# kekoveca/MPI-and-Open-MP

Measured on AMD Instinct MI355X. Metric: Gcell-updates/sec at 1/2/4/8 MI355X + % of HBM roofline, bit-exact, higher is better.
Workload: dtype u32 (1 bit/cell)

## Files before the change

include/life_mi355x.h:

```cpp
#ifndef LIFE_MI355X_H
#define LIFE_MI355X_H

#include <stdint.h>

#ifdef __cplusplus
extern "C" {
#endif

#define LIFE_OK 0
#define LIFE_EINVAL (-1)
#define LIFE_EHIP (-2)
#define LIFE_ERCCL (-3)
#define LIFE_ENOMEM (-4)
#define LIFE_ESTATE (-5)
#define LIFE_EIO (-6)

#define LIFE_KERNEL_BYTE 0
#define LIFE_KERNEL_BIT 1

#define LIFE_XPORT_AUTO 0
#define LIFE_XPORT_RCCL 1
#define LIFE_XPORT_LOCAL 2

typedef struct life_dev life_dev;
// ... 76 lines not shown

int life_dev_gather_bits(life_dev *d, uint8_t *packed);

int64_t life_dev_live_count(life_dev *d);

int life_dev_checksum(life_dev *d, uint64_t *sum);


int life_dev_clear(life_dev *d);

int life_dev_set_cells(life_dev *d, const int64_t *xy, int64_t n, int alive);

int life_dev_gather_rect(life_dev *d, int64_t x0, int64_t y0, int64_t w, int64_t h, uint8_t *cells);

int life_dev_gather_density(life_dev *d, int64_t fx, int64_t fy, uint32_t *counts);

int life_dev_sync(life_dev *d);
int life_dev_barrier(life_dev *d);
int life_device_count(void);
int life_dev_layout(life_dev *d, int local_shard, life_layout *out);
int life_dev_world(life_dev *d, int *world, int *dims0, int *dims1, int *nlocal, int *transport);
int life_dev_shard_info(life_dev *d, int local_shard, int *device, char pci_bus_id[64], int *rccl_nranks);

int life_dev_set_timing(life_dev *d, int on);

#define LIFE_OPT_SMALL_GRID 1
#define LIFE_OPT_OVERLAP 2
#define LIFE_OPT_BLOCK_GENS 5
#define LIFE_OPT_SMALL_WINDOW 4
#define LIFE_OPT_LOOPBACK 6
#define LIFE_OPT_FLOW 7
#define LIFE_OPT_FLOW_CHUNK 8
#define LIFE_OPT_DEEP_HALO 9
int life_dev_configure(life_dev *d, int option, int value);
#define LIFE_PATH_NONE 0
#define LIFE_PATH_ONEGEN 1
#define LIFE_PATH_TILES 2
#define LIFE_PATH_FLOW 3
#define LIFE_PATH_SMALL 5
int life_dev_last_path(life_dev *d);
int life_dev_kernel_stats(life_dev *d, double *avg_ms, int64_t *launches, double *bytes_per_launch);
int life_dev_kernel_work(life_dev *d, double *cell_updates_per_launch, double *valu_ops_per_launch);
int life_dev_phase_stats(life_dev *d, double *ring_ms, double *interior_ms, double *halo_ms, double *block_ms,
                         int64_t *blocks);
int life_dev_call_stats(life_dev *d, double *host_enqueue_ms, double *pass_enqueue_max_ms, int64_t *passes,
                        double *device_span_ms);

int life_tune(int kernel, int rows, int depth);

int life_tune_temporal(int kernel, int rows);

int life_measure_copy(int device, int64_t bytes, int reps, double *gbps);

void life_dev_destroy(life_dev *d);

#ifdef __cplusplus
}
#endif
#endif
```

mpi-and-open-mp_amd/csrc/life_dev.hip:

```cpp
#include <stdarg.h>

#include <chrono>
#include <thread>

#include "life_dev_internal.h"
#include "life_env.h"

using namespace life::rt;

thread_local std::string life::rt::g_err;

void life::rt::set_err(const char *fmt, ...) {
    char buf[512];
    va_list ap;
    va_start(ap, fmt);
    vsnprintf(buf, sizeof buf, fmt, ap);
    va_end(ap);
    g_err = buf;
}

static const int kEnvBlockGens = life::env::read(life::env::kBlockGens);
static const int kEnvFlow = life::env::read(life::env::kFlow);
static const bool kEnvDeepHalo = life::env::read(life::env::kDeepHalo) != 0;
static int default_block_gens(int kernel) {
    return kEnvBlockGens ? kEnvBlockGens : (kernel == LIFE_KERNEL_BIT ? 12 : 32);
}

namespace {

int alloc_fill_byte() { return life::env::read(life::env::kPoison) ? 0xA5 : 0; }

int shard_alloc(Shard &s) {
    HIPCHK(hipSetDevice(s.device));
    HIPCHK(hipStreamCreateWithPriority(&s.stream, hipStreamNonBlocking, 0));
    HIPCHK(hipStreamCreateWithPriority(&s.stream2, hipStreamNonBlocking, 0));
    HIPCHK(hipStreamCreateWithPriority(&s.comm_stream, hipStreamNonBlocking, 0));
    const int fill = alloc_fill_byte();
    const int64_t slack = s.lay.generations_per_exchange > 1 ? life::kTemporalSlackRows : 0;
    const size_t bytes = (size_t)(s.lay.pitch * (s.lay.rows + slack));
    for (int i = 0; i < 2; i++) {
        HIPCHK(hipMalloc(&s.buf[i], bytes));
        HIPCHK(hipMemsetAsync(s.buf[i], fill, bytes, s.stream));
    }
    HIPCHK(hipEventCreateWithFlags(&s.ev_int, hipEventDisableTiming));
    HIPCHK(hipEventCreateWithFlags(&s.ev_halo, hipEventDisableTiming));
    HIPCHK(hipEventCreateWithFlags(&s.ev_sync, hipEventDisableTiming));
    HIPCHK(hipEventCreateWithFlags(&s.ev_entry, hipEventDisableTiming));
    const size_t col_bytes = (size_t)life::column_stage_bytes(s.lay);
    HIPCHK(hipMalloc(&s.col_send, col_bytes));
    HIPCHK(hipMalloc(&s.col_recv, col_bytes));
    HIPCHK(hipMalloc(&s.d_count, 2 * sizeof(unsigned long long)));
    HIPCHK(hipMalloc(&s.sink, 1024));
    HIPCHK(hipMemsetAsync(s.col_send, fill, col_bytes, s.stream));
    HIPCHK(hipMemsetAsync(s.col_recv, fill, col_bytes, s.stream));
    HIPCHK(hipMemsetAsync(s.d_count, 0, 2 * sizeof(unsigned long long), s.stream));
    HIPCHK(hipMemsetAsync(s.sink, fill, 1024, s.stream));
    HIPCHK(hipStreamSynchronize(s.stream));
    HIPCHK(hipHostMalloc(&s.h_count, 2 * sizeof *s.h_count, hipHostMallocDefault));
    return LIFE_OK;
}

void shard_free(Shard &s) {
    (void)hipSetDevice(s.device);
    if (s.comm) (void)ncclCommDestroy(s.comm);
    for (auto &t : s.timers) {
        if (t.a) (void)hipEventDestroy(t.a);
        if (t.b) (void)hipEventDestroy(t.b);
    }
    for (auto &p : s.phases)
        for (hipEvent_t e : {p.ring0, p.ring1, p.int0, p.int1, p.halo0, p.halo1, p.end})
            if (e) (void)hipEventDestroy(e);
    for (uint8_t *p : {s.buf[0], s.buf[1], s.col_send, s.col_recv, s.sink, s.stage})
        if (p) (void)hipFree(p);
    if (s.flow) (void)hipFree(s.flow);
    if (s.d_count) (void)hipFree(s.d_count);
    if (s.h_count) (void)hipHostFree(s.h_count);
    for (hipEvent_t e : {s.ev_halo, s.ev_sync, s.ev_int, s.ev_entry, s.own_a, s.own_b})
        if (e) (void)hipEventDestroy(e);
    if (s.stream) (void)hipStreamDestroy(s.stream);
    if (s.stream2) (void)hipStreamDestroy(s.stream2);
    if (s.comm_stream) (void)hipStreamDestroy(s.comm_stream);
}

double comm_timeout_s() {
    static const double t = life::env::read(life::env::kCommTimeoutS);
    return t;
}

int agree_all_ranks(life_dev *d, int value, const char *what) {
    for (Shard &s : d->shards) {
        if (!s.comm) continue;
        HIPCHK(hipSetDevice(s.device));
        int64_t *h = reinterpret_cast<int64_t *>(s.h_count);
        h[0] = value;
        h[1] = -(int64_t)value;
        HIPCHK(hipMemcpyAsync(s.d_count, h, 2 * sizeof(int64_t), hipMemcpyHostToDevice, s.stream));
        NCCLCHK(ncclAllReduce(s.d_count, s.d_count, 2, ncclInt64, ncclMax, s.comm, s.stream));
        HIPCHK(hipMemcpyAsync(h, s.d_count, 2 * sizeof(int64_t), hipMemcpyDeviceToHost, s.stream));
        CHK(bounded_sync(s, what, -1));
        const int64_t hi = h[0], lo = -h[1];
        if (hi != lo) {
            set_err("%s is collective in rank mode: ranks passed %lld .. %lld", what, (long long)lo, (long long)hi);
            return LIFE_EINVAL;
        }
    }
    return LIFE_OK;
}

life_dev *new_dev(int64_t nx, int64_t ny, int dims0, int dims1, int world, int kernel) {
    int dims[2] = {dims0, dims1};
    if (dims0 <= 0 || dims1 <= 0) life_dims_create(world, dims);
    if (dims[0] * dims[1] != world) return nullptr;
    life_dev *d = new life_dev;
    d->nx = nx;
    d->ny = ny;
    d->dims[0] = dims[0];
    d->dims[1] = dims[1];
    d->world = world;
    d->kernel = kernel;
    d->block_gens = default_block_gens(kernel);
    d->deep = kEnvDeepHalo;
    d->flow = kEnvFlow;
    return d;
}

int create_shards(life_dev *d, const std::vector<int> &ranks, const std::vector<int> &devices) {
    for (size_t i = 0; i < ranks.size(); i++) {
        d->shards.emplace_back();
        Shard &s = d->shards.back();
        s.rank = ranks[i];
        s.device = devices[i];
        const int rc = life_layout_query(d->nx, d->ny, d->dims[0], d->dims[1], s.rank, d->kernel, &s.lay);
        if (rc != LIFE_OK) {
            set_err("layout: nx=%lld ny=%lld dims=%dx%d rank %d kernel %d", (long long)d->nx,
                    (long long)d->ny, d->dims[0], d->dims[1], s.rank, d->kernel);
            return rc;
        }
    }
    for (Shard &s : d->shards) CHK(shard_alloc(s));
    return plan_halos(d);
}

void tail_prewarm(const life_dev *d) {
    for (size_t i = 0; i < d->shards.size(); ++i) {
        bool seen = false;
        for (size_t j = 0; j < i; ++j)
            seen |= d->shards[j].lay.w == d->shards[i].lay.w && d->shards[j].lay.h == d->shards[i].lay.h;
        if (!seen) life::prewarm_tail_plans(d->shards[i].lay, max_pass_gens(d), part(d, 1));
    }
}

int finish_create(life_dev *d, int rc, life_dev **out) {
    if (rc != LIFE_OK) {
        life_dev_destroy(d);
        return rc;
// ... 232 lines not shown
    if (!d) return LIFE_EINVAL;
    CHK(life_dev_sync(d));
    switch (option) {
    case LIFE_OPT_SMALL_GRID:
        if (value < 0 || value > 4) return LIFE_EINVAL;
        d->small_mode = value;
        return LIFE_OK;
    case LIFE_OPT_SMALL_WINDOW: {
        const int R = value >> 8, K = value & 255;
        if (value != 0 && (K < 1 || R < 1 || R > 8 || R == 7)) return LIFE_EINVAL;
        if (value != 0 && life::reg_win_plan(d->shards[0].lay, R, K).blocks == 0) {
            set_err("small-grid window R=%d K=%d does not fit this grid", R, K);
            return LIFE_EINVAL;
        }
        d->win_rows = R;
        d->win_halo = K;
        return LIFE_OK;
    }
    case LIFE_OPT_OVERLAP: d->overlap = value != 0; return LIFE_OK;
    case LIFE_OPT_BLOCK_GENS:
        if (value < 0 || value > 32) return LIFE_EINVAL;
        d->block_gens = value > 0 ? value : default_block_gens(d->kernel);
        tail_prewarm(d);
        return LIFE_OK;
    case LIFE_OPT_FLOW:
        if (value < 0 || value > 3) return LIFE_EINVAL;
        d->flow = value;
        return LIFE_OK;
    case LIFE_OPT_DEEP_HALO:
        if (value < 0 || value > 1) return LIFE_EINVAL;
        if (d->rank_mode && d->world > 1) CHK(agree_all_ranks(d, value, "LIFE_OPT_DEEP_HALO"));
        d->deep = value != 0;
        return LIFE_OK;
    case LIFE_OPT_FLOW_CHUNK:
        if (value < 0) return LIFE_EINVAL;
        d->flow_chunk = value;
        return LIFE_OK;
    case LIFE_OPT_LOOPBACK: {
        if (value < 0 || value > 3) return LIFE_EINVAL;
        if (d->world != 1 || d->shards.size() != 1) {
            set_err("loopback needs a single-shard world (world %d, %zu local shards)", d->world, d->shards.size());
            return LIFE_EINVAL;
        }
        Shard &s = d->shards[0];
        if (value && (s.lay.h < s.lay.yapron || s.lay.w < s.lay.xapron)) {
            set_err("loopback: %lld x %lld cells < the %lld-column / %lld-row halo", (long long)s.lay.w,
                    (long long)s.lay.h, (long long)s.lay.xapron, (long long)s.lay.yapron);
            return LIFE_EINVAL;
        }
        if (value && d->transport == LIFE_XPORT_RCCL && !s.comm) {
            set_err("loopback over RCCL needs a communicator (life_dev_create_rank with a unique id, or "
                    "life_dev_create_ex with LIFE_XPORT_RCCL)");
            return LIFE_EINVAL;
        }
        d->loop = value == 0 ? 0 : value == 1 ? 3 : value == 2 ? 1 : 2;
        CHK(plan_halos(d));
        CHK(exchange(d, 0, false));
        tail_prewarm(d);
        return life_dev_sync(d);
    }
    default: return LIFE_EINVAL;
    }
}

int life_tune(int kernel, int rows, int depth) {
    if ((rows && rows != 16 && rows != 32 && rows != 64) ||
// ... 20 lines not shown
```

mpi-and-open-mp_amd/csrc/life_dev_internal.h:

```cpp
#pragma once
#include <rccl/rccl.h>
#include <stdio.h>
#include <string.h>

#include <algorithm>
#include <string>
#include <vector>

#include "life_host.h"
#include "life_io.h"
#include "life_kernels.h"
#include "life_mi355x.h"

#pragma GCC visibility push(hidden)

namespace life {
namespace rt {

extern thread_local std::string g_err;
void set_err(const char *fmt, ...);

#define HIPCHK(expr)                                                                          \
    do {                                                                                      \
        hipError_t e_ = (expr);                                                               \
        if (e_ != hipSuccess) {                                                               \
            life::rt::set_err("%s:%d %s: %s", __FILE__, __LINE__, #expr, hipGetErrorString(e_)); \
            return e_ == hipErrorOutOfMemory ? LIFE_ENOMEM : LIFE_EHIP;                       \
        }                                                                                     \
    } while (0)

#define NCCLCHK(expr)                                                                         \
    do {                                                                                      \
        ncclResult_t r_ = (expr);                                                             \
        if (r_ != ncclSuccess) {                                                              \
            life::rt::set_err("%s:%d %s: %s", __FILE__, __LINE__, #expr, ncclGetErrorString(r_)); \
            return LIFE_ERCCL;                                                                \
        }                                                                                     \
    } while (0)

#define CHK(expr)                     \
    do {                              \
        int rc_ = (expr);             \
        if (rc_ != LIFE_OK) return rc_; \
    } while (0)

struct TimedLaunch {
    hipEvent_t a = nullptr, b = nullptr;
    int launches = 1;
};

struct PhaseEvents {
    hipEvent_t ring0 = nullptr, ring1 = nullptr, int0 = nullptr, int1 = nullptr, halo0 = nullptr,
               halo1 = nullptr, end = nullptr;
};

struct LocalCopy {
    int phase, src, sop, sslot, dop, dslot;
    size_t bytes;
};

struct Shard {
    int rank = 0;
    int device = 0;
    life_layout lay{};
    uint8_t *buf[2] = {nullptr, nullptr};
    int cur = 0;
    hipStream_t stream = nullptr;
    hipStream_t stream2 = nullptr;
    hipStream_t comm_stream = nullptr;
    hipEvent_t ev_halo = nullptr, ev_sync = nullptr, ev_int = nullptr;
    hipEvent_t ev_entry = nullptr;
    hipEvent_t own_a = nullptr, own_b = nullptr, span_a = nullptr, span_b = nullptr;
    ncclComm_t comm = nullptr;
    uint8_t *col_send = nullptr, *col_recv = nullptr;
    unsigned long long *d_count = nullptr;
    unsigned long long *h_count = nullptr;
    uint8_t *sink = nullptr;
    uint8_t *stage = nullptr;
    size_t stage_bytes = 0;
    unsigned int *flow = nullptr;
    size_t flow_words = 0;
    bool flow_used = false;
    std::vector<life_halo_op> plan;
    bool corners = false;
    std::vector<int> slot;
    std::vector<LocalCopy> copies;
    std::vector<int> waits[2][2];
    std::vector<TimedLaunch> timers;
    size_t timers_used = 0;
    std::vector<PhaseEvents> phases;
    size_t phases_used = 0;
};

}
}

struct life_dev {
    int64_t nx = 0, ny = 0;
    int dims[2] = {1, 1};
    int world = 1;
    int kernel = LIFE_KERNEL_BYTE;
    int transport = LIFE_XPORT_LOCAL;
    bool rank_mode = false;
    bool timing = false;
    bool phase_events = true;
    bool launch_events = true;
    bool overlap = true;
    int block_gens = 0;
    int small_mode = 1;
    int win_rows = 0, win_halo = 0;
    int loop = 0;
    int last_path = LIFE_PATH_NONE;
    bool deep = true;
    int since = 0;
    int flow = 0;
    int64_t flow_chunk = 0;
    life::rt::TimedLaunch *call_timer = nullptr;
    std::vector<life::rt::Shard> shards;
    double acc_ms = 0.0;
    int64_t acc_launches = 0;
    double acc_bytes = 0.0;
    double acc_updates = 0.0;
    double acc_valu = 0.0;
    double ph_ring = 0.0, ph_int = 0.0, ph_halo = 0.0, ph_block = 0.0;
    int64_t ph_blocks = 0;
    double call_host_ms = 0.0, call_pass_max_ms = 0.0;
    int64_t call_passes = 0;
    bool call_spans = false;
};

namespace life {
namespace rt {

inline bool part(const life_dev *d, int a) { return d->dims[a] > 1 || ((d->loop >> a) & 1); }
inline bool self_wrap_x(const life_dev *d) { return !(d->loop & 1) && life::self_wrap_x(d->shards[0].lay, d->dims[0]); }
inline life::Wrap wrap_of(const life_dev *d) { return life::Wrap{!part(d, 0) && !self_wrap_x(d), !part(d, 1)}; }
inline bool temporal(const life_dev *d) { return d->shards[0].lay.generations_per_exchange > 1; }
inline bool deep_halo(const life_dev *d) {
    return d->deep && d->kernel == LIFE_KERNEL_BIT && temporal(d) && (part(d, 0) || part(d, 1)) && !self_wrap_x(d);
}
inline int max_pass_gens(const life_dev *d) {
    return std::min(std::min(d->shards[0].lay.generations_per_exchange, 32), d->block_gens);
}
inline Shard *find_local(life_dev *d, int rank) {
    for (Shard &s : d->shards)
        if (s.rank == rank) return &s;
    return nullptr;
}

// ... 27 lines not shown
```

mpi-and-open-mp_amd/csrc/life_env.h:

```cpp
#pragma once
#include <limits.h>
#include <stdlib.h>

#include "life_mi355x.h"

namespace life {
namespace env {

struct IntKnob { const char *name; int dflt, lo, hi; };
struct FlagKnob { const char *name; int dflt; };
struct RealKnob { const char *name; double dflt, lo, hi; };

inline int read(const IntKnob &k, int dflt) {
    const char *e = getenv(k.name);
    const int v = e ? atoi(e) : dflt;
    return v >= k.lo && v <= k.hi ? v : dflt;
}
inline int read(const IntKnob &k) { return read(k, k.dflt); }
inline int read(const FlagKnob &k) {
    const char *e = getenv(k.name);
    return e ? (atoi(e) != 0 ? 1 : 0) : k.dflt;
}
inline double read(const RealKnob &k) {
    const char *e = getenv(k.name);
    const double v = e ? atof(e) : k.dflt;
    return v > k.lo && v <= k.hi ? v : k.dflt;
}

constexpr IntKnob kStepRows{"LIFE_STEP_ROWS", 16, INT_MIN, INT_MAX};
constexpr IntKnob kStepDepth{"LIFE_STEP_DEPTH", 8, INT_MIN, INT_MAX};
constexpr FlagKnob kXcdOrderOnegen{"LIFE_XCD_ORDER_ONEGEN", -1};
constexpr IntKnob kTemporalRows{"LIFE_TEMPORAL_ROWS", 24, 16, 24};
constexpr IntKnob kTemporalRowsByte{"LIFE_TEMPORAL_ROWS_BYTE", 48, 32, 48};
constexpr FlagKnob kByteOneGhost{"LIFE_BYTE_ONE_GHOST", 1};
constexpr FlagKnob kBands{"LIFE_BANDS", 1};
constexpr FlagKnob kFlowBands{"LIFE_FLOW_BANDS", 1};
constexpr FlagKnob kXcdOrder{"LIFE_XCD_ORDER", 1};
constexpr FlagKnob kXcdOrderByte{"LIFE_XCD_ORDER_BYTE", 1};
constexpr IntKnob kTailSplit{"LIFE_TAIL_SPLIT", 2, 0, 2};
constexpr IntKnob kBlockGens{"LIFE_BLOCK_GENS", 0, 1, 32};
constexpr IntKnob kFlow{"LIFE_FLOW", 3, 0, 3};
constexpr FlagKnob kDeepHalo{"LIFE_DEEP_HALO", 1};
constexpr IntKnob kTimingMode{"LIFE_TIMING_MODE", 0, 0, 3};
constexpr FlagKnob kPoison{"LIFE_POISON", 0};
constexpr FlagKnob kInteriorTail{"LIFE_INTERIOR_TAIL", 0};
constexpr RealKnob kCommTimeoutS{"LIFE_COMM_TIMEOUT_S", 600.0, 0.0, 1e300};
constexpr IntKnob kTemporalDepth{"LIFE_TEMPORAL_DEPTH", LIFE_TEMPORAL_DEPTH, 1, 32};
constexpr IntKnob kTemporalDepthByte{"LIFE_TEMPORAL_DEPTH_BYTE", LIFE_TEMPORAL_DEPTH_BYTE, 1, 32};

}
}
```

mpi-and-open-mp_amd/csrc/life_host.h:

```cpp
#pragma once
#include <stdint.h>

#include "life_mi355x.h"

namespace life {

int halo_plan(int64_t nx, int64_t ny, int dims0, int dims1, int rank, int kernel, int loop, life_halo_op *ops,
              int max_ops);

#pragma GCC visibility push(hidden)
int halo_op_slot(const life_halo_op *ops, int i);
int halo_match_send(const life_halo_op *mine, int recv, int rank, const life_halo_op *peer_ops, int npeer);
int halo_wait_peers(const life_halo_op *ops, int n, int rank, int phase, int kind, int *peers);

struct PassPlan { int m; bool refill_first; bool extend; int ext; };
PassPlan next_pass(int K, int bmax, bool deep, int since, int64_t remaining);
#pragma GCC visibility pop

constexpr int64_t kFlowMaxHead = (int64_t)1 << 31;
int64_t flow_chunk_passes(int64_t tiles, int64_t grid, int64_t cap);

enum GatherFormat { kGatherDense = 0, kGatherVtk = 1, kGatherBits = 2 };
struct GatherPiece {
    int32_t rank;
    int32_t slot;
    int64_t bytes;
    int64_t row_bytes;
    int64_t rows;
    int64_t dst;
    int32_t shared_first;
    int32_t shared_last;
};
int64_t gather_frame_row_bytes(int64_t nx, int fmt);
int gather_plan(int64_t nx, int64_t ny, int dims0, int dims1, int kernel, int fmt, GatherPiece *pieces, int max,
                int64_t *slot_bytes);

struct TailPlan {
    int64_t F = 0, n2 = 0;
    double makespan = 0.0;
};
inline int64_t tail_row_items(int64_t ntx, int64_t B, int64_t rows) {
    return rows <= 0 ? 0 : B > 1 ? (ntx - 1) * rows + (rows + B - 1) / B : ntx * rows;
}
double tail_makespan2(int64_t ntx, int64_t B, int64_t F_rows, int64_t n2, int64_t slots, double c, int64_t pre = 0);
TailPlan tail_plan(int64_t ntx, int64_t B, int64_t ty0, int64_t ty1, int64_t yend, int64_t T, int64_t T2,
                   int64_t slots, int mode, double c, int64_t pre = 0);

}
```

mpi-and-open-mp_amd/csrc/life_plan.cpp:

```cpp
#include <stdio.h>
#include <stdlib.h>
#include <string.h>

#include <algorithm>
#include <mutex>
#include <vector>

#include "life_env.h"
#include "life_host.h"
#include "life_mi355x.h"

namespace {
constexpr int64_t kXoff = 128;
inline int64_t round_up(int64_t v, int64_t m) { return (v + m - 1) / m * m; }
inline int cart_rank(int c0, int c1, int dims1) { return c0 * dims1 + c1; }
}

extern "C" {

void life_decomposition(int64_t n, int p, int k, int64_t *start, int64_t *stop) {
    const int64_t l = n / p;
    *start = l * k;
    *stop = *start + l;
    if (k == p - 1) *stop = n;
// ... 76 lines not shown
    const int64_t xa = temporal_xapron(kernel);
    const bool temporal = K > 1 && temporal_ok(nx, ny, dims0, dims1, K, xa);
    out->xapron = temporal ? xa : 1;
    out->yapron = temporal ? K : 1;
    out->generations_per_exchange = temporal ? K : 1;
    const int64_t cells_per_unit = kernel == LIFE_KERNEL_BIT ? 128 : 16;
    out->units = (out->w + cells_per_unit - 1) / cells_per_unit;
    out->xoff = kXoff;
    out->pitch = round_up(kXoff + 16 * out->units + (temporal && kernel == LIFE_KERNEL_BYTE ? 64 : 16), 256);
    out->rows = out->h + 2 * out->yapron;
    return LIFE_OK;
}

}

int64_t life::flow_chunk_passes(int64_t tiles, int64_t grid, int64_t cap) {
    if (tiles < 1 || grid < 0 || cap < 0) return 0;
    int64_t n = (kFlowMaxHead - grid) / tiles;
    if (n < 0) n = 0;
    return cap > 0 && cap < n ? cap : n;
}

life::PassPlan life::next_pass(int K, int bmax, bool deep, int since, int64_t remaining) {
    int64_t seg = remaining;
    if (deep && since < K) seg = std::min(seg, (int64_t)(K - since));
    const int64_t n = (seg + bmax - 1) / bmax;
    PassPlan p;
    p.m = (int)((seg + n - 1) / n);
    p.refill_first = since + p.m > K;
    if (p.refill_first) since = 0;
    const bool last = remaining == p.m;
    p.extend = deep && since + p.m < K && !(last && since + p.m + bmax > K);
    p.ext = K - since - p.m;
    return p;
}

int life::halo_op_slot(const life_halo_op *ops, int i) {
    int n = 0;
    for (int k = 0; k < i; k++) n += ops[k].phase == ops[i].phase && ops[k].kind == ops[i].kind && ops[k].what == ops[i].what;
    return n;
}

int life::halo_match_send(const life_halo_op *mine, int recv, int rank, const life_halo_op *peer_ops, int npeer) {
    const life_halo_op &o = mine[recv];
    int kth = 0;
    for (int k = 0; k < recv; k++)
        kth += mine[k].phase == o.phase && mine[k].kind == LIFE_HALO_RECV && mine[k].peer == o.peer;
    for (int k = 0; k < npeer; k++) {
        const life_halo_op &q = peer_ops[k];
        if (q.phase == o.phase && q.kind == LIFE_HALO_SEND && q.peer == rank && kth-- == 0) return k;
    }
    return -1;
}

int life::halo_wait_peers(const life_halo_op *ops, int n, int rank, int phase, int kind, int *peers) {
    int ns = 0;
    for (int i = 0; i < n; i++) {
        if (ops[i].phase != phase || ops[i].kind != kind || ops[i].peer == rank) continue;
        if (std::find(peers, peers + ns, ops[i].peer) == peers + ns) peers[ns++] = ops[i].peer;
    }
    return ns;
}

int64_t life::gather_frame_row_bytes(int64_t nx, int fmt) {
    return fmt == kGatherBits ? (nx + 7) / 8 : nx * (fmt == kGatherVtk ? 2 : 1);
}
// ... 230 lines not shown
```

mpi-and-open-mp_amd/csrc/life_step.hip:

```cpp
#include <chrono>
#include <utility>

#include "life_dev_internal.h"
#include "life_env.h"

using namespace life::rt;

constexpr double kFlowAutoRounds = 5.0;
constexpr int64_t kFlowMinPasses = 4;

namespace {

int launch_region(life_dev *d, Shard &s, const life::Region &r, bool timed, hipStream_t st) {
    Bracket b;
    CHK(bracket_begin(d, s, timed, 1, kExtNever, false, st, &b));
    HIPCHK(life::launch_step(s.lay, s.buf[s.cur], s.buf[s.cur ^ 1], s.sink, r, wrap_of(d), st));
    CHK(bracket_end(b, st));
    if (b.t) {
        const bool bit = s.lay.kernel == LIFE_KERNEL_BIT;
        const int64_t cpu = bit ? 128 : 16;
        const int64_t xa = r.u0 * cpu, xb = r.u1 * cpu < s.lay.w ? r.u1 * cpu : s.lay.w;
        book(d, bit, (double)(xb - xa) * (double)(r.r1 - r.r0), 1.0, 1.0, 0.0);
    }
    return LIFE_OK;
}

int launch_tiles(life_dev *d, Shard &s, const life::TileRegion *r, int nreg, int m, bool timed, hipStream_t st,
                 life::Extend xt = life::Extend{}, int64_t concurrent = 0) {
    Bracket b;
    CHK(bracket_begin(d, s, timed, 1, kExtModeExt | kExtModeCall, false, st, &b));
    double valu = 0.0;
    HIPCHK(life::launch_tstep(s.lay, s.buf[s.cur], s.buf[s.cur ^ 1], r, nreg, m, wrap_of(d), st, &valu, b.ext_a,
                              b.ext_b, xt, concurrent));
    CHK(bracket_end(b, st));
    if (b.t) {
        const life::TileGeom g = life::tile_geom(life::extended_layout(s.lay, xt), m);
        double cells = 0.0;
        for (int k = 0; k < nreg; k++) {
            const int64_t xa = r[k].tx0 * g.lanes * g.cells, xb = std::min(r[k].tx1 * g.lanes * g.cells, s.lay.w);
            const int64_t ya = std::max(r[k].ty0 * g.rows - xt.y, (int64_t)0),
                          yb = std::min(r[k].ty1 * g.rows - xt.y, s.lay.h);
            if (xb > xa && yb > ya) cells += (double)(xb - xa) * (double)(yb - ya);
        }
        book(d, s.lay.kernel == LIFE_KERNEL_BIT, cells, (double)m, 1.0, valu);
    }
    return LIFE_OK;
}

bool interior_tail() { static const bool v = life::env::read(life::env::kInteriorTail) != 0; return v; }


int phase_begin(life_dev *d, Shard &s, PhaseEvents **pe) {
    *pe = nullptr;
    if (!d->timing || !d->phase_events) return LIFE_OK;
    int rc;
    *pe = phase_slot(s, &rc);
    if (!*pe) return rc;
    HIPCHK(hipEventRecord((*pe)->ring0, s.stream));
    return LIFE_OK;
}
int phase_ring(Shard &s, PhaseEvents *pe) {
    if (pe) {
        HIPCHK(hipEventRecord(pe->ring1, s.stream));
        HIPCHK(hipEventRecord(pe->halo0, s.stream));
    }
    return LIFE_OK;
}
int phase_end(life_dev *d, const std::vector<PhaseEvents *> &pe, const std::vector<char> &halo_side) {
    for (size_t si = 0; si < d->shards.size(); ++si) {
        Shard &s = d->shards[si];
        HIPCHK(hipSetDevice(s.device));
        if (pe[si]) HIPCHK(hipEventRecord(pe[si]->halo1, s.stream));
        if (halo_side[si]) {
            HIPCHK(hipEventRecord(s.ev_int, s.stream2));
            HIPCHK(hipStreamWaitEvent(s.stream, s.ev_int, 0));
        } else {
            HIPCHK(hipEventRecord(s.ev_halo, s.stream));
            HIPCHK(hipStreamWaitEvent(s.stream2, s.ev_halo, 0));
            std::swap(s.stream, s.stream2);
        }
        if (pe[si]) HIPCHK(hipEventRecord(pe[si]->end, s.stream));
// ... 24 lines not shown
        HIPCHK(hipEventRecord(s.ev_entry, s.stream));
        HIPCHK(hipStreamWaitEvent(s.stream2, s.ev_entry, 0));
        CHK(phase_begin(d, s, &pe[si]));
        CHK(ring(s));
        CHK(phase_ring(s, pe[si]));
        if (pe[si]) HIPCHK(hipEventRecord(pe[si]->int0, s.stream2));
        CHK(interior(s, &halo_side[si]));
        if (pe[si]) HIPCHK(hipEventRecord(pe[si]->int1, s.stream2));
    }
    CHK(exchange(d, 1, false));
    CHK(phase_end(d, pe, halo_side));
    for (Shard &s : d->shards) s.cur ^= 1;
    return LIFE_OK;
}

int generation_block(life_dev *d, const life::PassPlan &p) {
    const bool rx = part(d, 0) || self_wrap_x(d), ry = part(d, 1);
    const int m = p.m;
    if (p.refill_first) CHK(exchange(d, 0, false));
    if (p.extend) {
        life::Extend xt;
        xt.y = ry ? p.ext : 0;
        xt.x = part(d, 0);
        CHK(whole_block(d, false, [&](Shard &s) -> int {
            const life::TileGeom g = life::tile_geom(life::extended_layout(s.lay, xt), m);
            const life::TileRegion all{0, g.ntx, 0, g.nty};
            return launch_tiles(d, s, &all, 1, m, true, s.stream, xt);
        }));
        d->since += m;
        return LIFE_OK;
    }
    if (!(rx || ry) || !d->overlap)
        return whole_block(d, rx || ry, [&](Shard &s) -> int {
            const life::TileGeom g = life::tile_geom(s.lay, m);
            const life::TileRegion all{0, g.ntx, 0, g.nty};
            return launch_tiles(d, s, &all, 1, m, true, s.stream);
        });
    life::TileGeom g;
    life::TileRegion ring[4], inner;
    int n = 0;
    return overlapped_block(
        d,
        [&](Shard &s) -> int {
            const int64_t K = s.lay.generations_per_exchange;
            g = life::tile_geom(s.lay, m);
            const int64_t NX = g.ntx, NY = g.nty, uh = g.rows;
            int64_t ca = 0, cb = NX;
            if (rx) {
                ca = 1;
                cb = std::max(std::min(((s.lay.w - s.lay.xapron) / g.cells) / g.lanes, NX), ca);
            }
            int64_t ra = 0, rb = NY;
            if (ry) {
                ra = std::min((K + uh - 1) / uh, NY);
                rb = std::max(std::min((s.lay.h - K) / uh, NY), ra);
            }
            n = 0;
            if (ra > 0) ring[n++] = life::TileRegion{0, NX, 0, ra};
            if (rb < NY) ring[n++] = life::TileRegion{0, NX, rb, NY};
            if (rb > ra) {
                if (ca > 0) ring[n++] = life::TileRegion{0, ca, ra, rb};
                if (cb < NX) ring[n++] = life::TileRegion{cb, NX, ra, rb};
            }
            inner = life::TileRegion{ca, cb, ra, rb};
            return launch_tiles(d, s, ring, n, m, false, s.stream);
        },
// ... 92 lines not shown
}

int flow_form(const life_dev *d, int *m_out) {
    if (!d->flow || d->shards.size() != 1 || d->world != 1 || part(d, 0) || part(d, 1) || self_wrap_x(d) ||
        d->kernel != LIFE_KERNEL_BIT)
        return 0;
    const life_layout &L = d->shards[0].lay;
    const int m = max_pass_gens(d);
    *m_out = m;
    if (!life::flow_ok(L, m)) return 0;
    if (d->flow == 3) {
        const double rounds = (double)life::flow_items_per_pass(L, m) / (double)std::max(life::flow_slots(L), 1);
        return rounds < kFlowAutoRounds && !(rounds >= 1.0 && rounds < 1.5) ? 1 : 0;
    }
    return d->flow;
}

int flow_scratch(Shard &s, int m) {
    const life::TileGeom g = life::tile_geom(s.lay, m);
    const size_t words = (size_t)(2 + g.ntx * g.nty);
    if (words <= s.flow_words) return LIFE_OK;
    if (s.flow) (void)hipFree(s.flow);
    s.flow = nullptr;
    s.flow_words = 0;
    if (hipSetDevice(s.device) != hipSuccess || hipMalloc(&s.flow, words * sizeof(unsigned int)) != hipSuccess ||
        hipMemsetAsync(s.flow, 0, 2 * sizeof(unsigned int), s.stream) != hipSuccess) {
        set_err("dataflow scratch (%zu words)", words);
        return LIFE_ENOMEM;
    }
    s.flow_words = words;
    return LIFE_OK;
}

int step_flow(life_dev *d, int64_t generations, int64_t *done) {
    *done = 0;
    int m = 0;
    const int form = flow_form(d, &m);
    if (form == 0) return LIFE_OK;
    Shard &s = d->shards[0];
    const life_layout &L = s.lay;
    const int64_t passes = generations / m;
    if (passes < kFlowMinPasses) return LIFE_OK;
    CHK(flow_scratch(s, m));
    HIPCHK(hipSetDevice(s.device));
    const int64_t tiles = life::flow_items_per_pass(L, m);
    const int64_t per = life::flow_chunk_passes(tiles, life::flow_slots(L), d->flow_chunk);
    if (per < 1) return LIFE_OK;
    for (int64_t left = passes; left > 0;) {
        const int64_t n = std::min(left, per);
        Bracket b;
        CHK(bracket_begin(d, s, true, (int)n, kExtModeExt, false, s.stream, &b));
        HIPCHK(life::launch_tflow(L, s.buf[s.cur], s.buf[s.cur ^ 1], m, n, s.flow, s.flow + 2, wrap_of(d),
                                  form, s.stream, b.ext_a, b.ext_b));
        CHK(bracket_end(b, s.stream));
        if (b.t)
            book(d, true, (double)L.w * (double)L.h, (double)n * (double)m, (double)n,
                 (double)n * (double)life::flow_items_per_pass(L, m, true) * 64.0 *
                     life::tstep_valu_per_tile_lane(m, false));
        if (n & 1) s.cur ^= 1;
        left -= n;
    }
    s.flow_used = true;
    *done = passes * m;
    return LIFE_OK;
}

double ms_since(std::chrono::steady_clock::time_point t0) {
    return std::chrono::duration<double, std::milli>(std::chrono::steady_clock::now() - t0).count();
}
void note_pass(life_dev *d, std::chrono::steady_clock::time_point t0) {
    const double ms = ms_since(t0);
    d->call_passes++;
    if (ms > d->call_pass_max_ms) d->call_pass_max_ms = ms;
}

int step_body(life_dev *d, int64_t generations) {
    if (small_grid(d)) {
        d->last_path = LIFE_PATH_SMALL;
        constexpr int64_t kChunk = 1 << 20;
        for (int64_t g = 0; g < generations; g += kChunk)
            CHK(step_small(d, generations - g < kChunk ? generations - g : kChunk));
        return exchange(d, 0, false);
    }
    if (temporal(d)) {
        int64_t done = 0;
        CHK(step_flow(d, generations, &done));
        d->last_path = done > 0 ? LIFE_PATH_FLOW : LIFE_PATH_TILES;
        const int K = d->shards[0].lay.generations_per_exchange;
        for (int64_t g = done; g < generations;) {
            const life::PassPlan p = life::next_pass(K, max_pass_gens(d), deep_halo(d), d->since, generations - g);
            const auto t0 = std::chrono::steady_clock::now();
            CHK(generation_block(d, p));
            note_pass(d, t0);
            g += p.m;
        }
        return LIFE_OK;
    }
    d->last_path = LIFE_PATH_ONEGEN;
    for (int64_t g = 0; g < generations; g++) {
        const auto t0 = std::chrono::steady_clock::now();
        CHK(generation(d));
        note_pass(d, t0);
    }
    return LIFE_OK;
}

int step_call(life_dev *d, int64_t generations) {
    const bool one_stream = d->shards.size() == 1 && !part(d, 0) && !part(d, 1) && !self_wrap_x(d);
    for (Shard &s : d->shards) {
        if (one_stream) break;
        HIPCHK(hipSetDevice(s.device));
        HIPCHK(hipEventRecord(s.ev_entry, s.stream));
        HIPCHK(hipStreamWaitEvent(s.stream2, s.ev_entry, 0));
        HIPCHK(hipStreamWaitEvent(s.comm_stream, s.ev_entry, 0));
    }
    if (d->timing && one_stream && timing_mode() == kTimeCall && !small_grid(d) && temporal(d)) {
        Shard &s = d->shards[0];
        int rc;
        d->call_timer = timer_slot(s, &rc);
        if (!d->call_timer) return rc;
        d->call_timer->launches = 0;
        HIPCHK(hipEventRecord(d->call_timer->a, s.stream));
        rc = step_body(d, generations);
        TimedLaunch *t = d->call_timer;
        d->call_timer = nullptr;
        if (rc != LIFE_OK) {
            s.timers_used--;
            return rc;
        }
        HIPCHK(hipEventRecord(t->b, s.stream));
        s.span_a = t->a;
        s.span_b = t->b;
        d->call_spans = true;
        return LIFE_OK;
    }
    if (!d->timing) return step_body(d, generations);
    for (Shard &s : d->shards) {
        HIPCHK(hipSetDevice(s.device));
        if (!s.own_a) HIPCHK(hipEventCreate(&s.own_a));
        if (!s.own_b) HIPCHK(hipEventCreate(&s.own_b));
        HIPCHK(hipEventRecord(s.own_a, s.stream));
    }
    CHK(step_body(d, generations));
    for (Shard &s : d->shards) {
        HIPCHK(hipSetDevice(s.device));
        HIPCHK(hipEventRecord(s.own_b, s.stream));
        s.span_a = s.own_a;
        s.span_b = s.own_b;
    }
    d->call_spans = true;
    return LIFE_OK;
}

}

int life::rt::flow_prewarm(life_dev *d) {
    int m = 0;
    const int form = flow_form(d, &m);
    if (form == 0) return LIFE_OK;
    Shard &s = d->shards[0];
    CHK(flow_scratch(s, m));
    HIPCHK(hipSetDevice(s.device));
    HIPCHK(life::prewarm_tflow(s.lay, m, form, s.flow, s.stream));
    HIPCHK(hipStreamSynchronize(s.stream));
    return LIFE_OK;
}

extern "C" {

int life_dev_step(life_dev *d, int64_t generations) {
    if (!d || generations < 0) return LIFE_EINVAL;
    if (generations == 0) return LIFE_OK;
    const auto t0 = std::chrono::steady_clock::now();
    d->call_passes = 0;
    d->call_pass_max_ms = 0.0;
    d->call_spans = false;
// ... 9 lines not shown
```

mpi-and-open-mp_amd/life_mi355x/__init__.py:

```python
from __future__ import annotations

import ctypes
import importlib.abc
import os
import sys

import numpy as np

from .cfg import (bits_bytes, density_bytes, load_bits, load_cfg, load_cfg_cells, load_density,
                  save_vtk, vtk_bytes, vtk_header)

HERE = os.path.dirname(os.path.abspath(__file__))
LIB_PATH = os.environ.get("LIFE_MI355X_LIB") or os.path.join(HERE, "liblife_mi355x.so")

KERNEL_BYTE = 0
KERNEL_BIT = 1
KERNELS = {"byte": KERNEL_BYTE, "bit": KERNEL_BIT}
XPORT_AUTO, XPORT_RCCL, XPORT_LOCAL = 0, 1, 2
HALO_SEND, HALO_RECV, HALO_FILL = 0, 1, 2
HALO_COLUMN, HALO_ROW, HALO_CORNER = 0, 1, 2
OPT_SMALL_GRID, OPT_OVERLAP, OPT_SMALL_WINDOW, OPT_BLOCK_GENS, OPT_LOOPBACK, OPT_FLOW = 1, 2, 4, 5, 6, 7
OPT_FLOW_CHUNK = 8
OPT_DEEP_HALO = 9
TEMPORAL_DEPTH = {"bit": 32, "byte": 32}
BLOCK_GENS = {"bit": 12, "byte": 32}
TEMPORAL_ROWS = {"bit": 24, "byte": 48}
TILE_WAVES = {"bit": 8, "byte": 8}
TEMPORAL_XAPRON = {"bit": 64, "byte": 32}

ABI_SYMBOLS = (
    "life_decomposition", "life_dims_create", "life_dims_choose", "life_halo_plan", "life_layout_query",
    "life_strerror", "life_last_error", "life_dev_create", "life_dev_create_ex",
    "life_get_unique_id", "life_dev_create_rank", "life_dev_upload", "life_dev_fill_random",
    "life_dev_step", "life_dev_gather", "life_dev_live_count", "life_dev_sync",
    "life_dev_layout", "life_dev_world", "life_dev_set_timing", "life_dev_kernel_stats",
    "life_tune", "life_tune_temporal", "life_dev_configure", "life_dev_kernel_work", "life_dev_checksum",
    "life_dev_gather_vtk", "life_dev_gather_bits", "life_dev_destroy", "life_measure_copy", "life_dev_phase_stats",
    "life_dev_barrier", "life_device_count", "life_dev_last_path", "life_dev_call_stats",
    "life_dev_strerror", "life_dev_shard_info",
    "life_dev_clear", "life_dev_set_cells", "life_dev_gather_rect", "life_dev_gather_density",
)
PATHS = {0: "none", 1: "onegen", 2: "tiles", 3: "flow", 5: "small"}


class LifeError(RuntimeError):
    def __init__(self, rc: int, what: str):
        lib = _lib()
        detail = lib.life_last_error().decode(errors="replace")
        super().__init__(f"{what}: {lib.life_strerror(rc).decode()} ({rc}){': ' + detail if detail else ''}")
        self.rc = rc


class HaloOp(ctypes.Structure):
    _fields_ = [("phase", ctypes.c_int32), ("kind", ctypes.c_int32), ("peer", ctypes.c_int32),
                ("what", ctypes.c_int32), ("index", ctypes.c_int64), ("first", ctypes.c_int64),
                ("count", ctypes.c_int64), ("width", ctypes.c_int64)]
# ... 350 lines not shown
```

Measured before the change: 121,500.

## Pipeline temporal tile passes across two streams by row regions with event dependencies

Splits each temporal-blocked pass into R row regions launched alternately on two streams. Per-region events let a region of the next pass start once its neighbouring regions of the previous pass are done, instead of waiting for the whole pass to drain. The goal is to hide the tail and launch gaps between successive whole-grid kernel passes on a single device. It adds more launches and event traffic, and relies on a planner for correct cross-stream dependencies, which risks races or extra overhead on small grids.

```diff
diff --git a/include/life_mi355x.h b/include/life_mi355x.h
--- a/include/life_mi355x.h
+++ b/include/life_mi355x.h
@@ -132,6 +132,7 @@
 #define LIFE_OPT_FLOW 7
 #define LIFE_OPT_FLOW_CHUNK 8
 #define LIFE_OPT_DEEP_HALO 9
+#define LIFE_OPT_PIPELINE 11
 int life_dev_configure(life_dev *d, int option, int value);
 #define LIFE_PATH_NONE 0
 #define LIFE_PATH_ONEGEN 1
diff --git a/mpi-and-open-mp_amd/csrc/life_dev.hip b/mpi-and-open-mp_amd/csrc/life_dev.hip
--- a/mpi-and-open-mp_amd/csrc/life_dev.hip
+++ b/mpi-and-open-mp_amd/csrc/life_dev.hip
@@ -22,6 +22,10 @@
 static const int kEnvBlockGens = life::env::read(life::env::kBlockGens);
 static const int kEnvFlow = life::env::read(life::env::kFlow);
 static const bool kEnvDeepHalo = life::env::read(life::env::kDeepHalo) != 0;
+static const int kEnvPipeline = [] {
+    const int v = life::env::read(life::env::kPipeline);
+    return v == 2 ? life::env::kPipeline.dflt : v;
+}();
 static int default_block_gens(int kernel) {
     return kEnvBlockGens ? kEnvBlockGens : (kernel == LIFE_KERNEL_BIT ? 12 : 32);
 }
@@ -46,6 +50,7 @@
     HIPCHK(hipEventCreateWithFlags(&s.ev_halo, hipEventDisableTiming));
     HIPCHK(hipEventCreateWithFlags(&s.ev_sync, hipEventDisableTiming));
     HIPCHK(hipEventCreateWithFlags(&s.ev_entry, hipEventDisableTiming));
+    for (hipEvent_t &e : s.ev_pipe) HIPCHK(hipEventCreateWithFlags(&e, hipEventDisableTiming));
     const size_t col_bytes = (size_t)life::column_stage_bytes(s.lay);
     HIPCHK(hipMalloc(&s.col_send, col_bytes));
     HIPCHK(hipMalloc(&s.col_recv, col_bytes));
@@ -76,6 +81,8 @@
     if (s.d_count) (void)hipFree(s.d_count);
     if (s.h_count) (void)hipHostFree(s.h_count);
     for (hipEvent_t e : {s.ev_halo, s.ev_sync, s.ev_int, s.ev_entry, s.own_a, s.own_b})
+        if (e) (void)hipEventDestroy(e);
+    for (hipEvent_t e : s.ev_pipe)
         if (e) (void)hipEventDestroy(e);
     if (s.stream) (void)hipStreamDestroy(s.stream);
     if (s.stream2) (void)hipStreamDestroy(s.stream2);
@@ -121,6 +128,7 @@
     d->block_gens = default_block_gens(kernel);
     d->deep = kEnvDeepHalo;
     d->flow = kEnvFlow;
+    d->pipe = kEnvPipeline;
     return d;
 }
 
@@ -419,6 +427,10 @@
         if (d->rank_mode && d->world > 1) CHK(agree_all_ranks(d, value, "LIFE_OPT_DEEP_HALO"));
         d->deep = value != 0;
         return LIFE_OK;
+    case LIFE_OPT_PIPELINE:
+        if (value < 0 || value == 2 || value > life::kPipeMaxRegions) return LIFE_EINVAL;
+        d->pipe = value;
+        return LIFE_OK;
     case LIFE_OPT_FLOW_CHUNK:
         if (value < 0) return LIFE_EINVAL;
         d->flow_chunk = value;
diff --git a/mpi-and-open-mp_amd/csrc/life_dev_internal.h b/mpi-and-open-mp_amd/csrc/life_dev_internal.h
--- a/mpi-and-open-mp_amd/csrc/life_dev_internal.h
+++ b/mpi-and-open-mp_amd/csrc/life_dev_internal.h
@@ -44,6 +44,8 @@
         if (rc_ != LIFE_OK) return rc_; \
     } while (0)
 
+constexpr int kPipeRing = 2 * life::kPipeMaxRegions;
+
 struct TimedLaunch {
     hipEvent_t a = nullptr, b = nullptr;
     int launches = 1;
@@ -70,6 +72,7 @@
     hipStream_t comm_stream = nullptr;
     hipEvent_t ev_halo = nullptr, ev_sync = nullptr, ev_int = nullptr;
     hipEvent_t ev_entry = nullptr;
+    hipEvent_t ev_pipe[kPipeRing] = {};
     hipEvent_t own_a = nullptr, own_b = nullptr, span_a = nullptr, span_b = nullptr;
     ncclComm_t comm = nullptr;
     uint8_t *col_send = nullptr, *col_recv = nullptr;
@@ -115,6 +118,12 @@
     int since = 0;
     int flow = 0;
     int64_t flow_chunk = 0;
+    int pipe = 0;
+    struct {
+        int R = 0, m = 0;
+        int64_t pass = 0;
+        life::PipePlan plan;
+    } pipe_call;
     life::rt::TimedLaunch *call_timer = nullptr;
     std::vector<life::rt::Shard> shards;
     double acc_ms = 0.0;
diff --git a/mpi-and-open-mp_amd/csrc/life_env.h b/mpi-and-open-mp_amd/csrc/life_env.h
--- a/mpi-and-open-mp_amd/csrc/life_env.h
+++ b/mpi-and-open-mp_amd/csrc/life_env.h
@@ -41,6 +41,7 @@
 constexpr IntKnob kBlockGens{"LIFE_BLOCK_GENS", 0, 1, 32};
 constexpr IntKnob kFlow{"LIFE_FLOW", 3, 0, 3};
 constexpr FlagKnob kDeepHalo{"LIFE_DEEP_HALO", 1};
+constexpr IntKnob kPipeline{"LIFE_PIPELINE", 1, 0, 16};
 constexpr IntKnob kTimingMode{"LIFE_TIMING_MODE", 0, 0, 3};
 constexpr FlagKnob kPoison{"LIFE_POISON", 0};
 constexpr FlagKnob kInteriorTail{"LIFE_INTERIOR_TAIL", 0};
diff --git a/mpi-and-open-mp_amd/csrc/life_host.h b/mpi-and-open-mp_amd/csrc/life_host.h
--- a/mpi-and-open-mp_amd/csrc/life_host.h
+++ b/mpi-and-open-mp_amd/csrc/life_host.h
@@ -15,6 +15,17 @@
 
 struct PassPlan { int m; bool refill_first; bool extend; int ext; };
 PassPlan next_pass(int K, int bmax, bool deep, int since, int64_t remaining);
+
+constexpr int kPipeMaxRegions = 16, kPipeMaxStreams = 4;
+struct PipePlan {
+    int R = 0, S = 0;
+    bool aligned = false;
+    int64_t ty[kPipeMaxRegions + 1] = {};
+    int nwait[kPipeMaxRegions] = {};
+    int wait[kPipeMaxRegions][kPipeMaxStreams] = {};
+    bool record[kPipeMaxRegions] = {};
+};
+PipePlan pipe_plan(int64_t nty, int64_t B, int R, int S);
 #pragma GCC visibility pop
 
 constexpr int64_t kFlowMaxHead = (int64_t)1 << 31;
diff --git a/mpi-and-open-mp_amd/csrc/life_plan.cpp b/mpi-and-open-mp_amd/csrc/life_plan.cpp
--- a/mpi-and-open-mp_amd/csrc/life_plan.cpp
+++ b/mpi-and-open-mp_amd/csrc/life_plan.cpp
@@ -132,6 +132,38 @@
     const bool last = remaining == p.m;
     p.extend = deep && since + p.m < K && !(last && since + p.m + bmax > K);
     p.ext = K - since - p.m;
+    return p;
+}
+
+life::PipePlan life::pipe_plan(int64_t nty, int64_t B, int R, int S) {
+    PipePlan p;
+    if (R < 3 || R > kPipeMaxRegions || S < 1 || S > kPipeMaxStreams || nty < 2 * (int64_t)R) return p;
+    p.R = R;
+    p.S = S;
+    p.aligned = B > 1 && nty / B >= R;
+    const int64_t unit = p.aligned ? B : 1, units = nty / unit;
+    p.ty[0] = 0;
+    for (int r = 0; r < R; r++) p.ty[r + 1] = p.ty[r] + unit * (units / R + (r < units % R ? 1 : 0));
+    p.ty[R] = nty;
+    int know[2 * kPipeMaxRegions][kPipeMaxStreams];
+    for (int i = 0; i < 2 * R; i++) {
+        int *k = know[i];
+        for (int s = 0; s < S; s++) k[s] = i >= S ? know[i - S][s] : -1;
+        if (i >= S) k[i % S] = i - S;
+        if (i < R) continue;
+        const int j = i - R;
+        int need[3];
+        for (int dr = -1; dr <= 1; dr++) need[dr + 1] = ((j + dr + 1) % R + R) % R;
+        std::sort(need, need + 3, [](int a, int b) { return a > b; });
+        for (int q : need) {
+            if (k[q % S] >= q) continue;
+            p.wait[j][p.nwait[j]++] = i - q;
+            for (int s = 0; s < S; s++) k[s] = std::max(k[s], know[q][s]);
+            k[q % S] = std::max(k[q % S], q);
+        }
+    }
+    for (int j = 0; j < R; j++)
+        for (int w = 0; w < p.nwait[j]; w++) p.record[((j - p.wait[j][w]) % R + R) % R] = true;
     return p;
 }
 
diff --git a/mpi-and-open-mp_amd/csrc/life_step.hip b/mpi-and-open-mp_amd/csrc/life_step.hip
--- a/mpi-and-open-mp_amd/csrc/life_step.hip
+++ b/mpi-and-open-mp_amd/csrc/life_step.hip
@@ -47,6 +47,65 @@
     return LIFE_OK;
 }
 
+
+constexpr int kPipeAutoRegions = 4;
+constexpr double kPipeAutoRounds = 1.0;
+constexpr int64_t kPipeAutoPasses = 4;
+
+int64_t tile_bands(const life::TileGeom &g) { return g.gsh < 6 ? 64 >> g.gsh : 1; }
+
+int fence_stream2(Shard &s) {
+    HIPCHK(hipEventRecord(s.ev_entry, s.stream));
+    HIPCHK(hipStreamWaitEvent(s.stream2, s.ev_entry, 0));
+    return LIFE_OK;
+}
+int join_stream2(Shard &s) {
+    HIPCHK(hipEventRecord(s.ev_int, s.stream2));
+    HIPCHK(hipStreamWaitEvent(s.stream, s.ev_int, 0));
+    return LIFE_OK;
+}
+
+int pipelined_pass(life_dev *d, Shard &s, int m) {
+    auto &pc = d->pipe_call;
+    const life::TileGeom g = life::tile_geom(s.lay, m);
+    if (pc.m != m) {
+        if (pc.m != 0) {
+            CHK(join_stream2(s));
+            CHK(fence_stream2(s));
+        }
+        pc.plan = life::pipe_plan(g.nty, tile_bands(g), pc.R, 2);
+        pc.m = m;
+        pc.pass = 0;
+    }
+    const life::PipePlan &P = pc.plan;
+    if (P.R == 0) {
+        const life::TileRegion all{0, g.ntx, 0, g.nty};
+        return launch_tiles(d, s, &all, 1, m, true, s.stream);
+    }
+    Bracket b;
+    CHK(bracket_begin(d, s, true, 1, kExtNever, false, s.stream, &b));
+    hipStream_t st[2] = {s.stream, s.stream2};
+    double valu = 0.0;
+    for (int j = 0; j < P.R; j++) {
+        const int64_t i = pc.pass * P.R + j;
+        const int r = (int)((pc.pass + j) % P.R);
+        hipStream_t q = st[i % 2];
+        if (pc.pass > 0)
+            for (int w = 0; w < P.nwait[j]; w++)
+                HIPCHK(hipStreamWaitEvent(q, s.ev_pipe[(i - P.wait[j][w]) % kPipeRing], 0));
+        const life::TileRegion reg{0, g.ntx, P.ty[r], P.ty[r + 1]};
+        double v = 0.0;
+        HIPCHK(life::launch_tstep(s.lay, s.buf[s.cur], s.buf[s.cur ^ 1], &reg, 1, m, wrap_of(d), q, &v, nullptr,
+                                  nullptr, life::Extend{}, -1));
+        valu += v;
+        if (P.record[j]) HIPCHK(hipEventRecord(s.ev_pipe[i % kPipeRing], q));
+    }
+    CHK(bracket_end(b, s.stream));
+    if (b.t) book(d, s.lay.kernel == LIFE_KERNEL_BIT, (double)s.lay.w * (double)s.lay.h, (double)m, 1.0, valu);
+    pc.pass++;
+    return LIFE_OK;
+}
+
 bool interior_tail() { static const bool v = life::env::read(life::env::kInteriorTail) != 0; return v; }
 
 
@@ -137,6 +196,7 @@
     }
     if (!(rx || ry) || !d->overlap)
         return whole_block(d, rx || ry, [&](Shard &s) -> int {
+            if (d->pipe_call.R > 0) return pipelined_pass(d, s, m);
             const life::TileGeom g = life::tile_geom(s.lay, m);
             const life::TileRegion all{0, g.ntx, 0, g.nty};
             return launch_tiles(d, s, &all, 1, m, true, s.stream);
@@ -295,20 +355,26 @@
     return LIFE_OK;
 }
 
+int64_t flow_passes(const life_dev *d, int64_t generations, int *form, int *m, int64_t *per) {
+    *form = flow_form(d, m);
+    if (*form == 0) return 0;
+    const life_layout &L = d->shards[0].lay;
+    const int64_t passes = generations / *m;
+    if (passes < kFlowMinPasses) return 0;
+    *per = life::flow_chunk_passes(life::flow_items_per_pass(L, *m), life::flow_slots(L), d->flow_chunk);
+    return *per < 1 ? 0 : passes;
+}
+
 int step_flow(life_dev *d, int64_t generations, int64_t *done) {
     *done = 0;
-    int m = 0;
-    const int form = flow_form(d, &m);
-    if (form == 0) return LIFE_OK;
+    int m = 0, form = 0;
+    int64_t per = 0;
+    const int64_t passes = flow_passes(d, generations, &form, &m, &per);
+    if (passes == 0) return LIFE_OK;
     Shard &s = d->shards[0];
     const life_layout &L = s.lay;
-    const int64_t passes = generations / m;
-    if (passes < kFlowMinPasses) return LIFE_OK;
     CHK(flow_scratch(s, m));
     HIPCHK(hipSetDevice(s.device));
-    const int64_t tiles = life::flow_items_per_pass(L, m);
-    const int64_t per = life::flow_chunk_passes(tiles, life::flow_slots(L), d->flow_chunk);
-    if (per < 1) return LIFE_OK;
     for (int64_t left = passes; left > 0;) {
         const int64_t n = std::min(left, per);
         Bracket b;
@@ -368,8 +434,47 @@
     return LIFE_OK;
 }
 
+int pipe_regions(const life_dev *d, int64_t generations) {
+    if (d->pipe == 0 || d->shards.size() != 1 || d->world != 1 || part(d, 0) || part(d, 1) || self_wrap_x(d) ||
+        !temporal(d) || small_grid(d))
+        return 0;
+    if (d->timing && d->launch_events && timing_mode() != kTimeCall && timing_mode() != kTimeOff) return 0;
+    int form = 0, fm = 0;
+    int64_t per = 0;
+    const int64_t rest = generations - flow_passes(d, generations, &form, &fm, &per) * fm;
+    const int bmax = max_pass_gens(d);
+    const int64_t passes = (rest + bmax - 1) / bmax;
+    if (passes < 2) return 0;
+    const life_layout &L = d->shards[0].lay;
+    const life::TileGeom g = life::tile_geom(L, (int)((rest + passes - 1) / passes));
+    int R = d->pipe;
+    if (R == 1) {
+        R = kPipeAutoRegions;
+        const int slots = life::tile_slots(L);
+        if (passes < kPipeAutoPasses || slots < 1 ||
+            (double)life::region_items(g, life::TileRegion{0, g.ntx, 0, g.nty}) < kPipeAutoRounds * R * slots)
+            return 0;
+    }
+    return life::pipe_plan(g.nty, tile_bands(g), R, 2).R;
+}
+
+int call_body(life_dev *d, int64_t generations) {
+    const int rc = step_body(d, generations);
+    const bool piped = d->pipe_call.R > 0;
+    d->pipe_call.R = 0;
+    if (rc == LIFE_OK && piped) CHK(join_stream2(d->shards[0]));
+    return rc;
+}
+
 int step_call(life_dev *d, int64_t generations) {
     const bool one_stream = d->shards.size() == 1 && !part(d, 0) && !part(d, 1) && !self_wrap_x(d);
+    d->pipe_call.R = 0;
+    if (one_stream) {
+        HIPCHK(hipSetDevice(d->shards[0].device));
+        d->pipe_call.R = pipe_regions(d, generations);
+        d->pipe_call.m = 0;
+        if (d->pipe_call.R > 0) CHK(fence_stream2(d->shards[0]));
+    }
     for (Shard &s : d->shards) {
         if (one_stream) break;
         HIPCHK(hipSetDevice(s.device));
@@ -384,7 +489,7 @@
         if (!d->call_timer) return rc;
         d->call_timer->launches = 0;
         HIPCHK(hipEventRecord(d->call_timer->a, s.stream));
-        rc = step_body(d, generations);
+        rc = call_body(d, generations);
         TimedLaunch *t = d->call_timer;
         d->call_timer = nullptr;
         if (rc != LIFE_OK) {
@@ -397,14 +502,14 @@
         d->call_spans = true;
         return LIFE_OK;
     }
-    if (!d->timing) return step_body(d, generations);
+    if (!d->timing) return call_body(d, generations);
     for (Shard &s : d->shards) {
         HIPCHK(hipSetDevice(s.device));
         if (!s.own_a) HIPCHK(hipEventCreate(&s.own_a));
         if (!s.own_b) HIPCHK(hipEventCreate(&s.own_b));
         HIPCHK(hipEventRecord(s.own_a, s.stream));
     }
-    CHK(step_body(d, generations));
+    CHK(call_body(d, generations));
     for (Shard &s : d->shards) {
         HIPCHK(hipSetDevice(s.device));
         HIPCHK(hipEventRecord(s.own_b, s.stream));
diff --git a/mpi-and-open-mp_amd/life_mi355x/__init__.py b/mpi-and-open-mp_amd/life_mi355x/__init__.py
--- a/mpi-and-open-mp_amd/life_mi355x/__init__.py
+++ b/mpi-and-open-mp_amd/life_mi355x/__init__.py
@@ -22,6 +22,7 @@
 OPT_SMALL_GRID, OPT_OVERLAP, OPT_SMALL_WINDOW, OPT_BLOCK_GENS, OPT_LOOPBACK, OPT_FLOW = 1, 2, 4, 5, 6, 7
 OPT_FLOW_CHUNK = 8
 OPT_DEEP_HALO = 9
+OPT_PIPELINE = 11
 TEMPORAL_DEPTH = {"bit": 32, "byte": 32}
 BLOCK_GENS = {"bit": 12, "byte": 32}
 TEMPORAL_ROWS = {"bit": 24, "byte": 48}
diff --git a/profiles/pipeline/ab.py b/profiles/pipeline/ab.py
--- /dev/null
+++ b/profiles/pipeline/ab.py
@@ -0,0 +1,83 @@
+import json
+import os
+import subprocess
+import sys
+import time
+
+ROOT = os.path.dirname(os.path.dirname(os.path.dirname(os.path.abspath(__file__))))
+P = {"LIFE_MI355X_LIB": os.environ.get("LIFE_AB_PARENT_LIB", "")}
+
+
+def arms(name):
+    if name == "default":
+        one = [("parent", P, []), ("R4", {"LIFE_PIPELINE": "4"}, []), ("off", {"LIFE_PIPELINE": "0"}, []),
+               ("R6", {"LIFE_PIPELINE": "6"}, []), ("R3", {"LIFE_PIPELINE": "3"}, []),
+               ("R8", {"LIFE_PIPELINE": "8"}, [])]
+        return one * 4
+    if name == "m10":
+        one = [("parent_m10", dict(P, LIFE_BLOCK_GENS="10"), []),
+               ("R4_m10", {"LIFE_PIPELINE": "4", "LIFE_BLOCK_GENS": "10"}, []),
+               ("R6_m10", {"LIFE_PIPELINE": "6", "LIFE_BLOCK_GENS": "10"}, []),
+               ("parent", P, []), ("auto", {}, [])]
+        return one * 3
+    if name == "driver":
+        a = ["--steps", "20", "--warmup", "5"]
+        return [("parent", P, a), ("R4", {"LIFE_PIPELINE": "4"}, a), ("auto", {}, a)] * 4
+    if name == "half":
+        a = ["--shape", "32768x65536"]
+        return [("parent", P, a), ("auto", {}, a), ("parent_flow0", dict(P, LIFE_FLOW="0"), a),
+                ("R4_flow0", {"LIFE_PIPELINE": "4", "LIFE_FLOW": "0"}, a)] * 4
+    if name == "byte":
+        a = ["--kernel", "byte"]
+        return [("parent", P, a), ("R4", {"LIFE_PIPELINE": "4"}, a), ("auto", {}, a),
+                ("R3", {"LIFE_PIPELINE": "3"}, a)] * 3
+    if name == "lasttail":
+        V = {"LIFE_MI355X_LIB": os.environ.get("LIFE_AB_VARIANT_LIB", "")}
+        s4, d = ["--steps", "48"], ["--steps", "20", "--warmup", "5"]
+        return ([("whole_4pass", {}, s4), ("split_4pass", V, s4)] * 4 +
+                [("whole_R4_driver", {"LIFE_PIPELINE": "4"}, d), ("split_R4_driver", dict(V, LIFE_PIPELINE="4"), d)] * 4 +
+                [("whole", {}, []), ("split", V, [])] * 3)
+    if name == "passes":
+        out = []
+        for n in (4, 8, 16):
+            a = ["--steps", str(12 * n)]
+            out += [(f"parent_{n}pass", P, a), (f"auto_{n}pass", {}, a)] * 4
+        return out
+    if name == "final":
+        b, h, s4 = ["--kernel", "byte"], ["--kernel", "byte", "--shape", "32768x65536"], ["--steps", "48"]
+        d = ["--steps", "20", "--warmup", "5"]
+        return ([("parent", P, []), ("auto", {}, [])] * 4 + [("parent_byte", P, b), ("auto_byte", {}, b)] * 4 +
+                [("parent_byte_half", P, h), ("auto_byte_half", {}, h)] * 4 +
+                [("parent_4pass", P, s4), ("auto_4pass", {}, s4)] * 4 +
+                [("parent_driver", P, d), ("auto_driver", {}, d)] * 4)
+    raise SystemExit(f"unknown set {name}")
+
+
+def main():
+    name, path = sys.argv[1], sys.argv[2]
+    if not os.path.exists(P["LIFE_MI355X_LIB"]):
+        raise SystemExit("LIFE_AB_PARENT_LIB: the parent commit's liblife_mi355x.so")
+    with open(path, "a") as out:
+        for label, env, args in arms(name):
+            t0 = time.time()
+            try:
+                r = subprocess.run([sys.executable, os.path.join(ROOT, "bench.py"), *args],
+                                   env=dict(os.environ, **env), capture_output=True, text=True, timeout=150, cwd=ROOT)
+            except subprocess.TimeoutExpired:
+                print(f"{label}: time limit, stopping", flush=True)
+                return 1
+            lines = [ln for ln in r.stdout.splitlines() if ln.startswith("{")]
+            if r.returncode != 0 or len(lines) != 1:
+                print(f"{label}: rc {r.returncode}\n{r.stdout[-1500:]}\n{r.stderr[-1500:]}", flush=True)
+                return 1
+            j = json.loads(lines[0])
+            rec = dict(set=name, arm=label, value=j["value"], live=j.get("config", {}).get("live_cells_end"),
+                       ms_per_step=j.get("ms_per_step"), call=j.get("call"), wall_s=round(time.time() - t0, 1))
+            out.write(json.dumps(rec) + "\n")
+            out.flush()
+            print(f"{label:16s} {j['value']:10.3f} Gcell/s  span {j.get('call', {}).get('device_span_ms')} ms", flush=True)
+    return 0
+
+
+if __name__ == "__main__":
+    sys.exit(main())
diff --git a/profiles/pipeline/trace_summary.py b/profiles/pipeline/trace_summary.py
--- /dev/null
+++ b/profiles/pipeline/trace_summary.py
@@ -0,0 +1,31 @@
+import csv
+import sys
+
+
+def main(path, passes):
+    rows = [r for r in csv.DictReader(open(path)) if "tstep" in r["Kernel_Name"]]
+    rows.sort(key=lambda r: int(r["Start_Timestamp"]))
+    per = 1
+    k = [(int(r["Start_Timestamp"]), int(r["End_Timestamp"]), int(r["Grid_Size_X"]) // int(r["Workgroup_Size_X"]),
+          r["Queue_Id"]) for r in rows]
+    whole = max(g for _, _, g, _ in k)
+    tail = [x for x in k if x[2] < whole / 2]
+    if tail:
+        n = 0
+        while n < len(k) and k[-1 - n][2] < whole / 2:
+            n += 1
+        call, per = k[-n:], n // passes
+    else:
+        call = k[-passes:]
+    t0 = call[0][0]
+    print(f"{len(call)} launches, {per} per pass, queues {sorted(set(q for *_, q in call))}")
+    for i, (a, b, g, q) in enumerate(call):
+        prev_end = call[i - 1][1] if i else a
+        print(f"{i:3d} queue {q} items {g:5d} start {(a - t0) / 1e3:9.1f} us  dur {(b - a) / 1e3:7.1f} us  "
+              f"starts {(prev_end - a) / 1e3:7.1f} us before the previous launch ends")
+    span = (call[-1][1] - t0) / 1e3
+    print(f"span {span:.1f} us, {span / passes:.1f} us per pass")
+
+
+if __name__ == "__main__":
+    main(sys.argv[1], int(sys.argv[2]))
```

New measurement: 126,000 (median of 6 runs). +3.7%, better.
